# joshuaowalker/specimux

Hardware: AMD Instinct MI355X
Metric: reads/sec demultiplexed, 768-specimen ITS panel on 765k ONT-style reads (higher is better)
Workload: dtype u32

## Files before the change

### specimux_amd/csrc/smx_demux_tile.h

```cpp
#ifndef SMX_DEMUX_TILE_H
#define SMX_DEMUX_TILE_H
#include <hip/hip_runtime.h>
#include <stdint.h>
#include "smx_internal.h"
#include "smx_barcode_core.h"
#include "smx_align_core.h"
#include "smx_scorer.h"

namespace smx {

__device__ inline void wave_exclusive_scan(unsigned short *a, int n) {
    int lane = threadIdx.x & 63;
    int chunk = (n + 63) / 64;
    int lo = lane * chunk, hi = lo + chunk < n ? lo + chunk : n;
    int sum = 0;
    for (int i = lo; i < hi; i++) sum += a[i];
    int incl = sum;
    for (int d = 1; d < 64; d <<= 1) {
        int v = __shfl_up(incl, d, 64);
        if (lane >= d) incl += v;
    }
    int run = incl - sum;
    for (int i = lo; i < hi; i++) { int v = a[i]; a[i] = (unsigned short)run; run += v; }
    if (lane == 63) a[n] = (unsigned short)incl;
}

__device__ __forceinline__ int nth_location(const unsigned *mrow, int MW, int jstar, int loc_ord) {
    int seen = 0;
    for (int w = jstar >> 5; w < MW; w++) {
        unsigned word = mrow[w];
        if (w == (jstar >> 5)) word &= ~0u << (jstar & 31);
        int pc = __popc(word);
        if (seen + pc > loc_ord) {
            for (int t = loc_ord - seen; t > 0; t--) word &= word - 1;
            return w * 32 + __ffs(word) - 1;
        }
        seen += pc;
    }
    return -1;
}


template <typename PW, int NT, int BSV, int CM, int SP>
struct DemuxTile {
    static constexpr bool sp = SP != 0;
    static constexpr bool cmode = CM == 1;
    static constexpr bool redo = CM == 2;
    static constexpr int PWBITS = (int)sizeof(PW) * 8;
    unsigned char *lds;
    const DevPanel *P;
    const uint8_t *windows;
    const int32_t *lens;
    uint32_t n_reads;
    smx_op *ops, *extra;
    uint32_t extra_cap;
    uint32_t *n_extra;
    unsigned long long *counts;
    smx_hit *dbg_hits;
    int8_t *dbg_bdist;
    unsigned *tile_counter;
    const unsigned *pre;
    DemuxAux aux;
    int R, NP, NB, S, H, MW, maxB, need_starts, n_pbc, NPAIR, npmeta, use_slots, use_bs, ncand;
    TileLayout T;
    int CS, NPs, NBs, lNPs, lNBs, G, logG, MBW;
    int stride, kidx, pfmin, preorient, minlen, maxlen, lH, SW;
    unsigned Hmagic, hcmagic;
    uint32_t redo_ratio, n_tiles;
    bool cfilt, timing;
    unsigned long long *tacc, *dbg_phase;
    PW *ppeq, *prpeq;
    unsigned *bpeq, *bsre;
    unsigned char *lut, *codes;
    unsigned *namask;
    int *lensL, *ocnt;
    HitL *hits;
    unsigned *masks, *tieb, *bres, *dmask;
    int tstr;
    EntL *ents;
    int *etail;
    unsigned short *offsA, *offsB;
    unsigned short *queue;
    int *cumL;
    smx_op *opsL;
    int *aggr;
    unsigned short *hmap, *clist;
    unsigned long long *pmask, *hcand;
    LPanel LP;
    int tid, wave;
    uint32_t cur, r0, nxt;
    int par, nr, nh, nI;
    bool live;
    unsigned popped;
    bool pop_issued;
    int *lensC, *ocntC;
    bool prelisted;
    int nq, nE_pre;

    __device__ __forceinline__ void workgroup_done() {
        __builtin_amdgcn_fence(__ATOMIC_RELEASE, "workgroup");
        const unsigned prev = atomicAdd(tile_counter + 2, 1u);
        if (prev == gridDim.x - 1) {
            __threadfence();
            tile_counter[0] = 0; tile_counter[2] = 0;
            if (!cmode) {
                *n_extra = atomicAdd(tile_counter + 3, 0u);
                tile_counter[1] = 0; tile_counter[3] = 0;
            }
        }
    }
    __device__ __forceinline__ int divH(int x) const { return lH >= 0 ? (x >> lH) : (int)__umulhi((unsigned)x, Hmagic); }
    __device__ __forceinline__ void tile_span(uint32_t t, uint32_t &first, int &count) const {
        if (!redo) {
            first = t * (uint32_t)R;
            count = (int)((n_reads - first) < (uint32_t)R ? (n_reads - first) : (uint32_t)R);
        } else {
            const uint32_t seg = t / redo_ratio, sub = t - seg * redo_ratio;
            const uint32_t base = aux.ovf_list[seg] * (uint32_t)aux.Rc;
            const uint32_t end = base + (uint32_t)aux.Rc < n_reads ? base + (uint32_t)aux.Rc : n_reads;
            first = base + sub * (uint32_t)R;
            count = first < end ? (int)((end - first) < (uint32_t)R ? (end - first) : (uint32_t)R) : 0;
            if (count == 0) first = base;
        }
    }
    __device__ __forceinline__ void stamp(int i) {
        asm volatile("" : "+v"(tid));
        if (timing) { unsigned long long _t = clock64(); tacc[i] += _t - tacc[10]; tacc[10] = _t; }
    }

    __device__ __forceinline__ void pop_tile() {
        if (tid == 0) {
            unsigned off = 0;
            asm volatile("" : "+v"(off));
            popped = atomicAdd(tile_counter + off, 1u);
        }
        pop_issued = true;
    }

    __device__ __forceinline__ bool setup(unsigned char *lds_, const DevPanel *P_, const uint8_t *windows_, const int32_t *lens_,
                                          uint32_t n_reads_, int R_arg, smx_op *ops_, smx_op *extra_, uint32_t extra_cap_,
                                          uint32_t *n_extra_, unsigned long long *counts_, smx_hit *dbg_hits_, int8_t *dbg_bdist_arg,
                                          unsigned *tile_counter_, int use_slots_arg, const unsigned *pre_, const DemuxAux &aux_) {
        lds = lds_; P = P_; windows = windows_; lens = lens_; n_reads = n_reads_; ops = ops_; extra = extra_; extra_cap = extra_cap_;
        n_extra = n_extra_; counts = counts_; dbg_hits = dbg_hits_; tile_counter = tile_counter_; pre = pre_; aux = aux_;
        R = SP == 3 ? 32 : (SP == 2 ? SMX_SP2_R : (sp ? 64 : R_arg));
        NP = SP == 2 ? 2 : P->NP; NB = P->NB; S = SP == 3 ? 160 : (sp ? 80 : P->S); H = 2 * NP; MW = (S + 31) / 32; maxB = P->maxB;
        need_starts = sp ? 0 : P->need_starts;
        n_pbc = P->n_pbc; NPAIR = SP == 2 ? 1 : P->NPAIR;
        const LayoutArgs la = layout_args(NP, NB, n_pbc, NPAIR, P->trim);
        npmeta = la.npmeta;
        use_slots = SP != 0 ? 0 : use_slots_arg;
        dbg_bdist = SP != 0 ? nullptr : dbg_bdist_arg;
        use_bs = SP != 0 ? 1 : ((BSV != 0 && P->bs_ok && !use_slots) ? 1 : 0);
        ncand = la.ncand;
        const int tails = sp ? 0 : la.tails;
        T = make_layout<PW>(NP, NB, S, R, maxB, need_starts, npmeta, sp ? 3 : P->kidx, use_slots, P->bs_ok, ncand,
                            sp ? 0 : P->cap_hits, sp ? 0 : P->cap_ents, (sp && CM == 1) ? 256 : aux.nitems, tails, P->n_bstab);
        ppeq = (PW *)(lds + T.ppeq);
        prpeq = (PW *)(lds + T.prpeq);
        bpeq = (unsigned *)(lds + T.bpeq);
        bsre = (unsigned *)(lds + T.bsre);
        lut = lds + T.lut;
        codes = lds + T.codes;
        namask = (unsigned *)(lds + T.namask);
        lensL = (int *)(lds + T.lens);
        ocnt = (int *)(lds + T.ocnt);
        hits = (HitL *)(lds + T.hits);
        masks = (unsigned *)(lds + T.masks);
        if (layout_tie_in_rec(T.MBW, use_slots, tails)) { tieb = (unsigned *)(lds + T.hits); tstr = (int)(sizeof(HitL) / 4); }
        else { tieb = (unsigned *)(lds + T.tiem); tstr = sp ? 1 : T.MBW; }
        bres = (unsigned *)(lds + T.bres);
        dmask = (unsigned *)(lds + T.dmask);
        ents = (EntL *)(lds + T.ents);
        etail = (int *)(lds + T.etail);
        offsA = (unsigned short *)(lds + T.offsA);
        offsB = (unsigned short *)(lds + T.offsB);
        queue = (unsigned short *)(lds + T.queue);
        cumL = (int *)(lds + T.emit);
        opsL = (smx_op *)(lds + T.opsL);
        aggr = (int *)(lds + T.aggr);
        hmap = (unsigned short *)(lds + T.hmap);
        clist = (unsigned short *)(lds + T.clist);
        pmask = (unsigned long long *)(lds + T.pmask);
        hcand = (unsigned long long *)(lds + T.hcand);
        cfilt = layout_cfilt(H, NPAIR * 2);
        tid = threadIdx.x;
        wave = tid >> 6;
        if (redo && tile_counter[1] == 0) {
            if (tid == 0) workgroup_done();
            return false;
        }
        CS = T.CS; NPs = T.NPs; NBs = T.NBs; lNPs = T.lNPs; lNBs = T.lNBs; G = T.G; logG = T.logG; MBW = sp ? 1 : T.MBW;
        stride = SP == 3 ? 320 : (sp ? 160 : P->wstride);
        kidx = sp ? 3 : P->kidx; pfmin = P->pfmin;
        preorient = sp ? 1 : P->preorient; minlen = sp ? -1 : P->minlen; maxlen = sp ? -1 : P->maxlen;
        lH = (H & (H - 1)) == 0 ? 31 - __clz(H) : -1;
        Hmagic = (unsigned)((0x100000000ull + (unsigned)H - 1) / (unsigned)H);
        hcmagic = (unsigned)((0x100000000ull + (unsigned)(S >> 4) - 1) / (unsigned)((S >> 4) > 0 ? (S >> 4) : 1));
        redo_ratio = redo ? (uint32_t)((aux.Rc + R - 1) / R) : 1u;
        n_tiles = redo ? tile_counter[1] * redo_ratio : (n_reads + R - 1) / R;
        tacc = (unsigned long long *)(lds + T.tacc);
        dbg_phase = sp ? nullptr : P->dbg_phase;
        timing = dbg_phase != nullptr && tid == 0;
        SW = (R + 63) >> 6;
        return true;
    }

    __device__ __forceinline__ void stage_panel() {
        for (int i = tid; i < NP * 16; i += NT) {
            int p = i >> 4, c = i & 15;
            ppeq[c * NPs + p] = (PW)P->ppeq[i] << (PWBITS - P->pm[p]);
            if (need_starts) prpeq[c * NPs + p] = (PW)P->prpeq[i];
        }
        if (!use_bs)
            for (int i = tid; i < NB * 16; i += NT) bpeq[(i & 15) * NBs + (i >> 4)] = P->bpeq[i];
        if (use_bs)
            for (int i = tid; i < P->n_bstab * T.MBW * 256; i += NT) {
                int blk = i >> 8;
                bsre[blk * T.BSP + (i & 255)] = P->bs_re[i];
            }
        for (int i = tid; i < 512; i += NT) lut[i] = P->lut[i];
        int *pmeta = (int *)(lds + T.pmeta);
        {
            int *q = pmeta;
            LP.pm = q; q += NP; LP.pk = q; q += NP; LP.pdir = q; q += NP; LP.pfidx = q; q += NP;
            LP.pbc_off = q; q += NP + 1; LP.pbc = q; q += n_pbc; LP.bm = q; q += NB;
            LP.pair_f = q; q += NPAIR; LP.pair_r = q; q += NPAIR; LP.pair_pool = q; q += NPAIR;
            LP.bstab = q;
            for (int i = tid; i < NP; i += NT) q[i] = P->bs_tab[i];
            for (int i = tid; i < NP; i += NT) {
                pmeta[i] = P->pm[i]; pmeta[NP + i] = P->pk[i]; pmeta[2 * NP + i] = P->pdir[i]; pmeta[3 * NP + i] = P->pfidx[i];
            }
            for (int i = tid; i <= NP; i += NT) pmeta[4 * NP + i] = P->pbc_off[i];
            for (int i = tid; i < n_pbc; i += NT) pmeta[5 * NP + 1 + i] = P->pbc[i];
            for (int i = tid; i < NB; i += NT) pmeta[5 * NP + 1 + n_pbc + i] = P->bm[i];
            for (int i = tid; i < NPAIR; i += NT) {
                int *b = pmeta + 5 * NP + 1 + n_pbc + NB;
                b[i] = P->pair_f[i]; b[NPAIR + i] = P->pair_r[i]; b[2 * NPAIR + i] = P->pair_pool[i];
            }
        }
        if (tid < 12) aggr[tid] = 0;
        if (cfilt) for (int i = tid; i < R; i += NT) pmask[i] = 0ull;
        if (cfilt) for (int i = tid; i < H; i += NT) hcand[i] = 0ull;
        if (cmode && tid == 0) {
            HitL hn;
            hn.tail_end = -1; hn.nloc = 0; hn.ntied = 0; hn.first_tied = -1; hn.pdist = -1; hn.bbest = -2; hn.jstar = 0; hn.fs_j = 0;
            hn.flags = 0; hn.pad = 0;
            hits[T.NI] = hn;
            for (int w = 0; w < T.MBW; w++) tieb[T.NI * tstr + w] = 0;
        }
        __syncthreads();
        if (cfilt)
            for (int ci = tid; ci < NPAIR * 2; ci += NT) {
                const int pair = ci >> 1, o = ci & 1;
                const int h1 = LP.pair_f[pair] * 2 + (o == 0 ? 0 : 1), h2 = LP.pair_r[pair] * 2 + (o == 0 ? 1 : 0);
                atomicOr(&hcand[h1], 1ull << ci);
                atomicOr(&hcand[h2], 1ull << ci);
            }
        __syncthreads();

        if (timing) for (int i = 0; i < 11; i++) tacc[i] = 0;
    }

    __device__ __forceinline__ void primer_item(int item, const bool use_pre) {
        const int dn = cmode ? (int)clist[item] : item;
        int r = divH(dn), h = dn - __mul24(r, H), p = h >> 1, X = h & 1;
        int L = lensC[r];
        EndGeom g = end_geom(L, S);
        const unsigned char *cw = codes + __mul24(r * 2 + X, CS);
        const PW *peq = ppeq + p;
        const int m = LP.pm[p], k = LP.pk[p], top = PWBITS - 1;
        PW Pvv = ~(PW)0, Mv = 0;
        int score = m, best = m + 1, jstar = 0, cnt = 0;
        unsigned *mrow = masks + __mul24(item, MW);
        bool pre_done = false, pre_omatch = false;
        if (use_pre) {
            const uint32_t gr = r0 + (uint32_t)r;
            const unsigned *pw = pre + ((size_t)(gr >> 10) * H + h) * (S >> 4) * PRE_TILE + (gr & (PRE_TILE - 1));
            const int bfull = S == 160 ? prescan_decode<10>(pw, PRE_TILE, 10, MW, m, k, g.Sp, mrow, &jstar, &cnt)
                            : S == 80 ? prescan_decode<5>(pw, PRE_TILE, 5, MW, m, k, g.Sp, mrow, &jstar, &cnt)
                                      : prescan_decode<0>(pw, PRE_TILE, S >> 4, MW, m, k, g.Sp, mrow, &jstar, &cnt);
            pre_omatch = bfull <= k;
            if (g.j_lo == 0) { pre_done = true; best = pre_omatch ? bfull : m + 1; }
            else { jstar = 0; cnt = 0; }
        }
        if (pre_done) {
        } else if (sizeof(PW) == 4 && g.j_lo == 0 && g.Sp == S && (S & 3) == 0) {
            const unsigned *pq = (const unsigned *)ppeq + p;
            unsigned Pu = ~0u, Mu = 0;
            int sc = m, bst = m + 1;
            const int esh = lNPs + 2;
#define SMX_PCOL(J) do { const unsigned e_ = *(const unsigned *)((const char *)pq + ((unsigned)cw[J] << esh)); \
                     myers_step_hw_top(e_, Pu, Mu, sc);                                              \
                     ltw = __builtin_amdgcn_alignbit(ltw, (unsigned)(sc - bst), 31);                  \
                     gtw = __builtin_amdgcn_alignbit(gtw, (unsigned)(bst - sc), 31);                  \
                     bst = sc < bst ? sc : bst; } while (0)
            for (int w = 0; w < MW; w++) {
                const int ncols = S - w * 32 < 32 ? S - w * 32 : 32;
                unsigned gtw = 0, ltw = 0;
                int j = w * 32;
                const int jend = j + ncols;
                for (; j + 8 <= jend; j += 8) {
                    SMX_PCOL(j); SMX_PCOL(j + 1); SMX_PCOL(j + 2); SMX_PCOL(j + 3);
                    SMX_PCOL(j + 4); SMX_PCOL(j + 5); SMX_PCOL(j + 6); SMX_PCOL(j + 7);
                }
                if (j < jend) { SMX_PCOL(j); SMX_PCOL(j + 1); SMX_PCOL(j + 2); SMX_PCOL(j + 3); }
                if (ncols > 0) {
                    mrow[w] = __brev(~gtw) >> (32 - ncols);
                    if (ltw) jstar = w * 32 + ncols - __ffs(ltw);
                } else mrow[w] = 0;
            }
#undef SMX_PCOL
            best = bst; score = sc;
            Pvv = (PW)Pu; Mv = (PW)Mu;
            for (int w = jstar >> 5; w < MW; w++) {
                unsigned word = mrow[w];
                if (w == (jstar >> 5)) word &= ~0u << (jstar & 31);
                cnt += __popc(word);
            }
        } else if (g.j_lo == 0) {
            const int Sp = g.Sp;
            for (int w = 0; w < MW; w++) {
                unsigned word = 0;
                int jend = (w + 1) * 32 < Sp ? (w + 1) * 32 : Sp;
#pragma unroll 4
                for (int j = w * 32; j < jend; j++) {
                    myers_step<PW, false>(peq[(int)cw[j] << lNPs], Pvv, Mv, score, top);
                    bool lt = score < best;
                    best = lt ? score : best;
                    jstar = lt ? j : jstar;
                    word |= (score == best ? 1u : 0u) << (j & 31);
                }
                mrow[w] = word;
            }
            for (int w = jstar >> 5; w < MW; w++) {
                unsigned word = mrow[w];
                if (w == (jstar >> 5)) word &= ~0u << (jstar & 31);
                cnt += __popc(word);
            }
        } else {
            for (int w = 0; w < MW; w++) mrow[w] = 0;
            for (int j = g.j_lo; j < g.Sp; j++) {
                myers_step<PW, false>(peq[(int)cw[j] << lNPs], Pvv, Mv, score, top);
                if (score < best) { best = score; jstar = j; cnt = 0; }
                if (score == best) { cnt++; mrow[j >> 5] |= 1u << (j & 31); }
            }
        }
        bool matched = best <= k;
        bool omatch = matched;
        if (g.j_lo > 0 && use_pre) omatch = pre_omatch;
        else if (g.j_lo > 0) {
            PW P2 = ~(PW)0, M2 = 0;
            int sc = m, b2 = m + 1;
            for (int j = 0; j < g.Sp; j++) {
                myers_step<PW, false>(peq[(int)cw[j] << lNPs], P2, M2, sc, top);
                b2 = sc < b2 ? sc : b2;
            }
            omatch = b2 <= k;
        }
        int fs_j = jstar;
        if (matched && need_starts) {
            const PW *rpeq = prpeq + p;
            PW P2 = ~(PW)0, M2 = 0;
            int sc = m, lastc = 1;
            int maxc = m + best;
            for (int c = 1; c <= maxc; c++) {
                int j = jstar - (c - 1);
                if (j < g.j_lo) break;
                myers_step<PW, true>(rpeq[(int)cw[j] << lNPs], P2, M2, sc, m - 1);
                if (sc == best) lastc = c;
            }
            fs_j = jstar - (lastc - 1);
        }
        HitL hl;
        hl.tail_end = -1;
        hl.pdist = (signed char)(matched ? best : -1);
        hl.nloc = (short)(matched ? cnt : 0);
        hl.bbest = -2; hl.ntied = 0; hl.first_tied = -1;
        hl.jstar = (unsigned char)jstar; hl.fs_j = (unsigned char)fs_j;
        hl.flags = (unsigned char)(omatch ? 1 : 0); hl.pad = 0;
        hits[item] = hl;
        if (cfilt && matched) atomicOr(&pmask[r], 1ull << h);
        if (omatch) {
            int dir = LP.pdir[p];
            int vote_fwd = (dir == 0) ? (X == 0) : (X == 1);
            atomicAdd(&ocntC[r], vote_fwd ? 1 : 0x10000);
        }
    }

    __device__ __forceinline__ void phase2_primers() {
        unsigned short *fbq = queue;
        if (cmode) {
            for (int i0 = tid; i0 < nh; i0 += 4 * NT) {
                unsigned mw[4];
#pragma unroll
                for (int u = 0; u < 4; u++) {
                    const int i = i0 + u * NT < nh ? i0 + u * NT : nh - 1;
                    const int r = divH(i), h = i - __mul24(r, H);
                    const uint32_t gr = r0 + (uint32_t)r;
                    mw[u] = aux.match[((size_t)(gr >> 10) * H + h) * PRE_G + ((gr & (PRE_TILE - 1)) >> 5)] >> (gr & 31);
                }
#pragma unroll
                for (int u = 0; u < 4; u++) {
                    const int i = i0 + u * NT;
                    if (i < nh) {
                        const bool flagged = (mw[u] & 1u) || (ocntC[divH(i)] & OCNT_NA) != 0;
                        int rec = T.NI;
                        if (flagged) {
                            const int sl = atomicAdd(&aggr[11], 1);
                            if (sl < T.NI) { clist[sl] = (unsigned short)i; rec = sl; }
                        }
                        hmap[i] = (unsigned short)rec;
                    }
                }
            }
            __syncthreads();
            nI = aggr[11];
            if (nI > T.NI) {
                live = false;
                if (tid == 0) aux.ovf_list[atomicAdd(tile_counter + 1, 1u)] = cur;
            }
        }
        if (!live) {
        } else if (pre != nullptr) {
            for (int item = tid; item < nI; item += NT) {
                if ((ocntC[divH(cmode ? (int)clist[item] : item)] & OCNT_NA) == 0) primer_item(item, true);
                else fbq[atomicAdd(&aggr[10], 1)] = (unsigned short)item;
            }
            __syncthreads();
            const int nfb = aggr[10];
            if (nfb > 0) {
                for (int i = tid; i < nfb; i += NT) primer_item((int)fbq[i], false);
                __syncthreads();
                if (tid == 0) aggr[10] = 0;
            }
        } else {
            for (int item = tid; item < nI; item += NT) primer_item(item, false);
            __syncthreads();
        }

    }

    __device__ __forceinline__ int locations_needed(int item) {
        const int dn = cmode ? (int)clist[item] : item;
        int r = divH(dn), h = dn - __mul24(r, H), p = h >> 1, X = h & 1;
        int L = lensC[r];
        int f = ocntC[r] & 0x7FFF, rv = ocntC[r] >> 16;
        int ori = 3;
        if (preorient) { if (f > 0 && rv == 0) ori = 1; else if (rv > 0 && f == 0) ori = 2; }
        bool filtered = (minlen != -1 && L < minlen) || (maxlen != -1 && L > maxlen);
        int dir = LP.pdir[p];
        bool in_fwd = (dir == 0) ? (X == 0) : (X == 1);
        bool needed = !filtered && ((in_fwd && (ori & 1)) || (!in_fwd && (ori & 2)));
        HitL &hl = hits[item];
        int n = 0;
        if (needed && hl.pdist >= 0) {
            hl.flags |= 2;
            hl.bbest = -1;
            n = hl.nloc;
        }
        for (int w = 0; w < MBW; w++) tieb[__mul24(item, tstr) + w] = 0;
        return n;
    }
    __device__ __forceinline__ void list_entries(int item, int rank_in_round, int e) {
        const int dn = cmode ? (int)clist[item] : item;
        int r = divH(dn), h = dn - __mul24(r, H), X = h & 1;
        const HitL &hl = hits[item];
        int L = lensC[r];
        EndGeom g = end_geom(L, S);
        const unsigned *mrow = masks + __mul24(item, MW);
        const unsigned *na = namask + __mul24(r * 2 + X, MW);
        int ord = 0;
        for (int w = hl.jstar >> 5; w < MW; w++) {
            unsigned word = mrow[w];
            if (w == (hl.jstar >> 5)) word &= ~0u << (hl.jstar & 31);
            while (word) {
                int je = w * 32 + __ffs(word) - 1;
                word &= word - 1;
                int bstart = (je - g.j_lo) + g.shift + 1;
                BcGeom bg = bc_geom(L, g.base, bstart);
                int ncol = g.Sp - bg.tj0;
                bool ok = ncol > 0;
                if (ok && pfmin > 0) {
                    if (!bg.pf_same || ncol < pfmin) ok = false;
                    else {
                        int wi = bg.tj0 >> 5, sh = bg.tj0 & 31;
                        unsigned long long two = ((unsigned long long)(wi + 1 < MW ? na[wi + 1] : 0u) << 32) | na[wi];
                        if ((two >> sh) & ((1ull << pfmin) - 1ull)) ok = false;
                    }
                }
                EntL en;
                en.hit = (unsigned short)item;
                en.slot = (unsigned short)(rank_in_round << logG);
                en.tj0 = (unsigned char)(ok ? bg.tj0 : 0);
                en.loc_ord = (unsigned char)ord;
                en.ncol = (unsigned char)(ncol > 255 ? 255 : (ncol < 0 ? 0 : ncol));
                en.ok = ok ? 1 : 0;
                en.delta = (short)bg.delta; en.pad = 0;
                ents[e++] = en;
                ord++;
            }
        }
    }

    __device__ __forceinline__ void phase3a_entries() {
        if (dbg_bdist)
            for (int i = tid; i < nh * maxB; i += NT) dbg_bdist[(size_t)r0 * H * maxB + i] = -1;
        prelisted = false;
        nq = 0; nE_pre = 0;
        if (nI <= NT) {
            const int item = tid;
            const int n = item < nI ? locations_needed(item) : 0;
            const unsigned pk = (unsigned)n | ((n > 0 ? 1u : 0u) << 16);
            unsigned incl = pk;
            for (int d = 1; d < 64; d <<= 1) {
                unsigned v = (unsigned)__shfl_up((int)incl, d, 64);
                if ((tid & 63) >= d) incl += v;
            }
            unsigned *wsum = (unsigned *)offsB;
            if ((tid & 63) == 63) wsum[wave] = incl;
            __syncthreads();
            unsigned base = 0, total = 0;
            for (int w = 0; w < NT / 64; w++) { unsigned v = wsum[w]; total += v; base += w < wave ? v : 0u; }
            const unsigned excl = base + incl - pk;
            nq = (int)(total >> 16);
            const int totE = (int)(total & 0xFFFFu);
            if (nq <= T.CAPH && totE <= T.CAPE) {
                prelisted = true;
                nE_pre = totE;
                if (n > 0) {
                    queue[excl >> 16] = (unsigned short)item;
                    if (BSV == 3) offsA[item] = (unsigned short)(excl & 0xFFFFu);
                    list_entries(item, (int)(excl >> 16), (int)(excl & 0xFFFFu));
                }
                if (use_slots) { for (int i = tid; i < (nq << logG); i += NT) bres[i] = 0xFFFFFFFFu; }
                else { for (int i = tid; i < nq * (kidx + 1) * MBW; i += NT) dmask[i] = 0; }
                __syncthreads();
            } else {
                __syncthreads();
                if (item < nI) {
                    offsA[item] = (unsigned short)(excl & 0xFFFFu);
                    offsB[item] = (unsigned short)(excl >> 16);
                    if (n > 0) queue[excl >> 16] = (unsigned short)item;
                }
                if (tid == 0) { offsA[nI] = (unsigned short)totE; offsB[nI] = (unsigned short)nq; }
                __syncthreads();
            }
        } else {
            for (int item = tid; item < nI; item += NT) {
                int n = locations_needed(item);
                offsA[item] = (unsigned short)n;
                offsB[item] = n > 0 ? 1 : 0;
            }
            __syncthreads();
            if (wave == 0) wave_exclusive_scan(offsA, nI);
            else if (wave == 1) wave_exclusive_scan(offsB, nI);
            __syncthreads();
            for (int item = tid; item < nI; item += NT)
                if (offsB[item + 1] != offsB[item]) queue[offsB[item]] = (unsigned short)item;
            nq = offsB[nI];
            __syncthreads();
        }

    }

    __device__ __forceinline__ void phase3b_barcodes(int nE) {
        if (BSV != 0 && use_bs) {
            const int bsm = P->bs_m;
            for (int item = tid; item < nE * MBW; item += NT) {
                int ei = item, w = 0;
                if (MBW != 1) { ei = item / MBW; w = item - ei * MBW; }
                const EntL en = ents[ei];
                if (BSV == 3) etail[ei] = -0x7FFFFFFF;
                if (!en.ok) continue;
                const int hh = cmode ? (int)clist[en.hit] : (int)en.hit, r = divH(hh), h = hh - __mul24(r, H), p = h >> 1, X = h & 1;
                const unsigned char *cwt = codes + __mul24(r * 2 + X, CS) + en.tj0;
                unsigned *dm = dmask + __mul24(__mul24(en.slot >> logG, kidx + 1), MBW) + w;
                if constexpr (BSV == 3) {
                    unsigned seen[4], ML[4];
                    const unsigned want[4] = {~0u, ~0u, ~0u, ~0u};
                    int tc = -1;
// ... 214 lines not shown
                else {
                    if (tid == 0) aggr[8] = q0 + 1;
                    __syncthreads();
                    for (int q = q0 + 2 + tid; q <= nq && q - q0 <= T.CAPH; q += NT) {
                        const int hq = queue[q - 1];
                        if (offsA[hq] + hits[hq].nloc - e_base <= T.CAPE) atomicMax(&aggr[8], q);
                    }
                    __syncthreads();
                    q1 = aggr[8];
                }
                const int e_end = (q1 < nq) ? offsA[queue[q1]] : offsA[nI];
                nE = e_end - e_base;
                for (int q = q0 + tid; q < q1; q += NT) {
                    int item = queue[q];
                    list_entries(item, q - q0, offsA[item] - e_base);
                }
                if (use_slots) { for (int i = tid; i < ((q1 - q0) << logG); i += NT) bres[i] = 0xFFFFFFFFu; }
                else { for (int i = tid; i < (q1 - q0) * (kidx + 1) * MBW; i += NT) dmask[i] = 0; }
                __syncthreads();
            }
            stamp(3);
            if (!pop_issued) pop_tile();
            phase3b_barcodes(nE);
            __syncthreads();
            stamp(4);
            phase3c_summary(q0, q1, e_base);
            __syncthreads();
            stamp(5);
            q0 = q1;
        }
    }

    __device__ __forceinline__ void zero_for_next() {
        for (int i = tid; i < R * 2 * MW; i += NT) namask[i] = 0;
        for (int i = tid; i < R; i += NT) ocnt[(par ^ 1) * R + i] = 0;
        if (live) for (int i = tid; i < nr * ncand; i += NT) cumL[i] = 0;
        if (tid == 0) { aggr[9] = (int)popped; aggr[11] = 0; }
        __syncthreads();
        nxt = (uint32_t)aggr[9];

    }

    __device__ __forceinline__ void phase4_score() {
        unsigned long long t_sc0 = 0;
        if (timing) t_sc0 = clock64();
        const int lG = R <= 16 ? 2 : (R <= 32 ? 1 : 0), G = 1 << lG;
        const int r = tid >> lG, sub = tid & (G - 1);
        if (r < nr) {
            int L = lensC[r];
            bool filtered = (minlen != -1 && L < minlen) || (maxlen != -1 && L > maxlen);
            const unsigned long long pm_r = cfilt ? pmask[r] : 0ull;
            if (cfilt && sub == 0) pmask[r] = 0ull;
            if (sub == 0) atomicAdd(&aggr[0], 1);
            if (filtered) {
                if (sub == 0) {
                    atomicAdd(&aggr[2], 1);
                    smx_op op;
                    op.sample = -1; op.trim_start = 0; op.trim_end = 0; op.pool = -1; op.p1 = op.p2 = -1; op.barcode = -1;
                    op.dist[0] = op.dist[1] = op.dist[2] = op.dist[3] = -1;
                    op.rtype = SMX_R_FILTERED; op.flags = 0; op.n_ops = 0; op.read = r0 + r;
                    opsL[r] = op;
                }
            } else {
                ReadCtx c;
                c.P = P; c.LP = LP; c.MBW = MBW; c.L = L; c.S = S;
                c.trim = sp ? (int)SMX_TRIM_BARCODES : P->trim; c.derep = sp ? (int)SMX_DEREP_BEST : P->derep;
                c.npair = NPAIR;
                c.tstr = tstr;
                if (cmode) { c.hits = hits; c.tiem = tieb; c.hmap = hmap + r * H; }
                else { c.hits = hits + r * H; c.tiem = tieb + r * H * tstr; c.hmap = nullptr; }
                c.hcand = cfilt ? hcand : nullptr;
                c.pm = pm_r;
                c.g = end_geom(L, S);
                int f = ocntC[r] & 0x7FFF, rv = ocntC[r] >> 16;
                int ori = 3;
                if (preorient) { if (f > 0 && rv == 0) ori = 1; else if (rv > 0 && f == 0) ori = 2; }
                c.set_live(ori);
                Emitter E;
                E.c = &c; E.primary = opsL + r; E.extra = extra; E.extra_cap = extra_cap;
                E.n_extra = tile_counter + 3;
                E.counts = counts; E.cum = cumL + r * ncand; E.aggr = aggr; E.read = r0 + r;
                E.n = 0; E.matched = false; E.overflow = false;
                const bool done = score_fast(E, ori, sub, G);
                if (sub == 0) {
                    if (!done) score_general(E, ori);
                    opsL[r].n_ops = (uint16_t)E.n;
                    if (E.matched) atomicAdd(&aggr[1], 1);
                    if (E.n > 1) atomicAdd(&aggr[6], 1);
                    if (E.overflow) atomicAdd(&aggr[7], 1);
                }
            }
        }
        if (timing) tacc[9] += clock64() - t_sc0;

    }

    __device__ __forceinline__ void phase1_encode() {
        const int wid = live ? tid - 64 * SW : tid, nw = live ? NT - 64 * SW : NT;
        const bool timing_enc = dbg_phase != nullptr && tid == 64 * SW;
        unsigned long long t_enc0 = 0;
        if (timing_enc) t_enc0 = clock64();
        uint32_t r0n;
        int nrn;
        tile_span(nxt, r0n, nrn);
        int *lensN = lensL + (par ^ 1) * R;
        int len_n = 0;
        bool have_len = false;
        auto load_len = [&](int r_item) {
            unsigned off = r0n + (uint32_t)(wid < nrn ? wid : r_item);
            asm volatile("" : "+v"(off));
            return lens[off];
        };
        auto encode_bytes = [&](int r, int L, int cpos, const uint4 &v) {
            int Sp = L < S ? L : S;
            unsigned w[4] = {v.x, v.y, v.z, v.w};
            unsigned char *rowA = codes + (r * 2 + 0) * CS, *rowB = codes + (r * 2 + 1) * CS;
            for (int b = 0; b < 16; b++) {
                int pos = cpos + b;
                unsigned ch = (w[b >> 2] >> ((b & 3) * 8)) & 0xFF;
                if (pos < S) {
                    if (pos < Sp) {
                        unsigned cd = lut[256 + ch];
                        int j = Sp - 1 - pos;
                        rowA[j] = (unsigned char)cd;
                        if (cd > 3) { atomicOr(&namask[(r * 2 + 0) * MW + (j >> 5)], 1u << (j & 31)); atomicOr(&ocnt[(par ^ 1) * R + r], OCNT_NA); }
                    }
                } else if (pos < 2 * S) {
                    int j = pos - S;
                    if (j < Sp) {
                        unsigned cd = lut[ch];
                        rowB[j] = (unsigned char)cd;
                        if (cd > 3) { atomicOr(&namask[(r * 2 + 1) * MW + (j >> 5)], 1u << (j & 31)); atomicOr(&ocnt[(par ^ 1) * R + r], OCNT_NA); }
                    }
                }
            }
        };
        if ((S & 15) == 0 && (sp || aux.codes2 != nullptr)) {
            const int hc = S >> 4, per = 2 * hc;
            const bool tiled = SP == 2 ? true : aux.tiled != 0;
            auto fast = [&](int r, int end, int c, unsigned z) {
                unsigned *dst = (unsigned *)(codes + __mul24(r * 2 + end, CS)) + 4 * c;
#pragma unroll
                for (int q = 0; q < 4; q++) {
                    const unsigned x = (z >> (2 * q)) & 0x03030303u;
                    dst[q] = x ^ ((x >> 1) & 0x01010101u);
                }
            };
            auto slow = [&](int r, int end, int c) {
                const uint4 v = *(const uint4 *)(windows + (size_t)(r0n + r) * stride + (end ? S : 0) + 16 * c);
                encode_bytes(r, lens[r0n + r], (end ? S : 0) + 16 * c, v);
            };
            if (tiled && ((r0n | (uint32_t)nrn) & 3u) == 0) {
                const int nq = nrn >> 2;
                for (int ci = wid; ci < per * 16; ci += nw) {
                    const int run = ci >> 4, r = (ci & 15) * 4;
                    len_n = load_len(0);
                    have_len = true;
                    if ((ci & 15) >= nq) continue;
                    const int end = run >= hc ? 1 : 0, c = run - (end ? hc : 0);
                    uint4 z4 = *(const uint4 *)(aux.codes2 + tilecodes_word((size_t)(r0n + r), hc, end, c));
                    unsigned f4 = *(const unsigned *)(aux.naflag + r0n + r);
                    asm volatile("" : "+v"(z4.x), "+v"(z4.y), "+v"(z4.z), "+v"(z4.w), "+v"(f4), "+v"(len_n));
                    if (!(f4 & 0xFFu)) fast(r, end, c, z4.x);
                    if (!(f4 & 0xFF00u)) fast(r + 1, end, c, z4.y);
                    if (!(f4 & 0xFF0000u)) fast(r + 2, end, c, z4.z);
                    if (!(f4 & 0xFF000000u)) fast(r + 3, end, c, z4.w);
                    if (f4) {
#pragma nounroll
                        for (int j = 0; j < 4; j++)
                            if ((f4 >> (8 * j)) & 0xFFu) slow(r + j, end, c);
                    }
                }
            } else {
                const unsigned permagic = (unsigned)((0x100000000ull + (unsigned)per - 1) / (unsigned)per);
                const int nci = tiled ? per * 64 : nrn * per;
                auto item_of = [&](int ci, int &r, int &end, int &c) {
                    int rem;
                    if (tiled) { r = ci & 63; rem = ci >> 6; }
                    else { r = (int)__umulhi((unsigned)ci, permagic); rem = ci - __mul24(r, per); }
                    end = rem >= hc ? 1 : 0; c = rem - (end ? hc : 0);
                    return ci < nci && r < nrn;
                };
                for (int ci0 = wid; ci0 < nci; ci0 += 4 * nw) {
                    unsigned z[4], fl[4];
#pragma unroll
                    for (int u = 0; u < 4; u++) {
                        const int ci = ci0 + u * nw;
                        int r, end, c;
                        if (!item_of(ci, r, end, c)) r = end = c = 0;
                        z[u] = aux.codes2[tiled ? tilecodes_word((size_t)(r0n + r), hc, end, c) : (size_t)r0n * per + (size_t)(__mul24(r, per) + end * hc + c)];
                        fl[u] = aux.naflag[r0n + r];
                        if (u == 0) len_n = load_len(r);
                    }
                    have_len = true;
                    asm volatile("" : "+v"(z[0]), "+v"(z[1]), "+v"(z[2]), "+v"(z[3]), "+v"(fl[0]), "+v"(fl[1]), "+v"(fl[2]), "+v"(fl[3]), "+v"(len_n));
                    unsigned slow_u = 0;
#pragma unroll
                    for (int u = 0; u < 4; u++) {
                        int r, end, c;
                        if (!item_of(ci0 + u * nw, r, end, c)) continue;
                        if (!fl[u]) fast(r, end, c, z[u]);
                        else slow_u |= 1u << u;
                    }
#pragma nounroll
                    for (; slow_u; slow_u &= slow_u - 1u) {
                        int r, end, c;
                        item_of(ci0 + (__ffs((int)slow_u) - 1) * nw, r, end, c);
                        slow(r, end, c);
                    }
                }
            }
        } else if (!sp && (S & 15) == 0) {
            const int hc = S >> 4, nhead = nrn * hc, S4 = S >> 2;
            for (int ci = wid; ci < 2 * nhead; ci += nw) {
                const bool tail = ci >= nhead;
                const int k = tail ? ci - nhead : ci;
                const int r = hc == 1 ? k : (int)__umulhi((unsigned)k, hcmagic), c = k - __mul24(r, hc);
                const uint4 v = *(const uint4 *)(windows + (size_t)(r0n + r) * stride + (tail ? S : 0) + 16 * c);
                const int L = lens[r0n + r];
                const unsigned w[4] = {v.x, v.y, v.z, v.w};
                unsigned pk[4];
                bool acgt = L >= S;
#pragma unroll
                for (int q = 0; q < 4; q++) {
                    const unsigned x = (w[q] >> 1) & 0x03030303u;
                    const unsigned y = x ^ ((x >> 1) & 0x01010101u);
                    acgt = acgt && (__builtin_amdgcn_perm(0u, 0x54474341u, y) == w[q]);
                    pk[q] = tail ? y : __builtin_amdgcn_perm(0u, y ^ 0x03030303u, 0x00010203u);
                }
                if (acgt) {
                    unsigned *dst = (unsigned *)(codes + __mul24(r * 2 + (tail ? 1 : 0), CS));
#pragma unroll
                    for (int q = 0; q < 4; q++) dst[tail ? 4 * c + q : S4 - 1 - (4 * c + q)] = pk[q];
                } else {
                    encode_bytes(r, L, (tail ? S : 0) + 16 * c, v);
                }
            }
        } else if (!sp) {
            const int chunks = stride / 16;
            const uint4 *src = (const uint4 *)(windows + (size_t)r0n * stride);
            for (int ci = wid; ci < nrn * chunks; ci += nw) {
                int r = ci / chunks;
                encode_bytes(r, lens[r0n + r], (ci - r * chunks) * 16, src[ci]);
            }
        }
        if (wid < nrn) {
            if (!have_len) len_n = lens[r0n + wid];
            lensN[wid] = len_n;
        }
        if (timing_enc) tacc[8] += clock64() - t_enc0;
    }

    __device__ __forceinline__ void phase5_store() {
        if (live) {
            const uint4 *srcv = (const uint4 *)opsL;
            uint4 *dstv = (uint4 *)(ops + r0);
            for (int i = tid; i < nr * 2; i += NT) dstv[i] = srcv[i];
        }
        if (live && dbg_hits) {
            for (int item = tid; item < nh; item += NT) {
                int r = divH(item);
                const HitL &hl = hits[cmode ? (int)hmap[item] : item];
                EndGeom g = end_geom(lensC[r], S);
                smx_hit o;
                o.pdist = hl.pdist; o.nloc = hl.nloc;
                o.first_start = hl.pdist >= 0 ? (int)hl.fs_j - g.j_lo + g.shift : -1;
                o.first_end = hl.pdist >= 0 ? (int)hl.jstar - g.j_lo + g.shift : -1;
                o.bbest = hl.bbest; o.ntied = hl.ntied;
                o.first_tied = (short)((hl.bbest >= 0) ? LP.pbc[LP.pbc_off[(item - r * H) >> 1] + hl.first_tied] : -1);
                o.tail_end = (hl.bbest >= 0 && tstr != (int)(sizeof(HitL) / 4)) ? hl.tail_end : -1;
                o.flags = (int16_t)(hl.flags & 1);
                dbg_hits[(size_t)(r0 + r) * H + (item - r * H)] = o;
            }
        }
        if (dbg_hits) __syncthreads();

    }

    __device__ __forceinline__ void run() {
        cur = 0xFFFFFFFFu;
        par = 1;
        for (;;) {
            asm volatile("" : "+v"(tid));
            const bool have = cur != 0xFFFFFFFFu;
            popped = 0;
            pop_issued = false;
            r0 = 0u;
            nr = 0;
            if (have) tile_span(cur, r0, nr);
            nh = nr * H;
            nI = nh;
            live = have;
            lensC = lensL + par * R; ocntC = ocnt + par * R;
            if (timing) tacc[10] = clock64();
            if (have) {
                phase2_primers();
                stamp(1);
                if (live) {
                    phase3a_entries();
                    stamp(2);
                    phase3_rounds();
                }
            }
            if (!pop_issued) pop_tile();
            zero_for_next();
            stamp(0);
            if (live && wave < SW) phase4_score();
            else if (nxt < n_tiles) phase1_encode();
            __syncthreads();
            stamp(6);
            phase5_store();
            stamp(7);
            if (nxt >= n_tiles) break;
            cur = nxt;
            par ^= 1;
        }
    }

    __device__ __forceinline__ void finish() {
        if (timing)
            for (int i = 0; i < 10; i++) dbg_phase[(size_t)blockIdx.x * 16 + i] += tacc[i];
        if (timing) dbg_phase[(size_t)blockIdx.x * 16 + 14] += tacc[0] != 0 || tacc[1] != 0 ? 1 : 0;
        if (dbg_phase != nullptr && (tid & 63) == 0)
            dbg_phase[(size_t)blockIdx.x * 16 + 10 + wave] = __builtin_amdgcn_s_getreg(4 | (0 << 6) | (31 << 11));
    #undef STAMP
        if (tid < 8 && aggr[tid]) atomicAdd(&counts[tid], (unsigned long long)aggr[tid]);
        __syncthreads();
        if (tid == 0) workgroup_done();

    }
};

template <typename PW, int NT, int BSV, int CM = 0, int SP = 0>
__global__ __launch_bounds__(NT, SP == 2 ? SMX_SP2_WG : 4) void demux_kernel(DevPanel Pv, const uint8_t *__restrict__ windows,
                                                    const int32_t *__restrict__ lens, uint32_t n_reads, int R_arg,
                                                    smx_op *__restrict__ ops, smx_op *__restrict__ extra,
                                                    uint32_t extra_cap, uint32_t *n_extra,
                                                    unsigned long long *counts, smx_hit *dbg_hits, int8_t *dbg_bdist_arg,
                                                    unsigned *tile_counter, int use_slots_arg,
                                                    const unsigned *__restrict__ pre, uint32_t npad, DemuxAux aux) {
    extern __shared__ __attribute__((aligned(16))) unsigned char lds[];
    (void)npad;
    DemuxTile<PW, NT, BSV, CM, SP> D;
    if (!D.setup(lds, &Pv, windows, lens, n_reads, R_arg, ops, extra, extra_cap, n_extra, counts, dbg_hits, dbg_bdist_arg,
                 tile_counter, use_slots_arg, pre, aux))
        return;
    D.stage_panel();
    D.run();
    D.finish();
}

}
#endif
```

### specimux_amd/csrc/smx_prescan_core.h

```cpp
#ifndef SMX_PRESCAN_CORE_H
#define SMX_PRESCAN_CORE_H
#include <stdint.h>

#include "smx_hd.h"
#include "smx_bitslice_core.h"

namespace smx {

constexpr int PRE_G = 32;
constexpr int PRE_TILE = PRE_G * 32;
constexpr int PRE_MAXROWS = 31;
constexpr int PRE_MAXSYM = 8;
constexpr int PRE_BLK = 33;
constexpr int PRE_SUBG = 8;
constexpr int PRE_CS = 291;
static_assert(PRE_CS >= PRE_SUBG * PRE_BLK && PRE_CS % 32 == 3, "staging stride");
constexpr int PRE_SCRATCH = 2 * (PRE_MAXSYM + 1) * 64;

struct PreDesc {
    int NP, S, nsym, pure4;
    uint8_t m[64], k[64];
    uint8_t symmask[64][PRE_MAXSYM];
    uint8_t sym[64][32];
};

SMX_HD unsigned perm_b32(unsigned a, unsigned b, unsigned sel) {
#if defined(__HIP_DEVICE_COMPILE__)
    return __builtin_amdgcn_perm(a, b, sel);
#else
    unsigned r = 0;
    for (int i = 0; i < 4; i++) {
        const unsigned q = (sel >> (8 * i)) & 7u;
        r |= (((q & 4u) ? a : b) >> (8 * (q & 3u)) & 0xFFu) << (8 * i);
    }
    return r;
#endif
}

SMX_HD unsigned bfi_b32(unsigned mask, unsigned a, unsigned b) {
#if defined(__HIP_DEVICE_COMPILE__)
    unsigned r;
    asm("v_bfi_b32 %0, %1, %2, %3" : "=v"(r) : "s"(mask), "v"(a), "v"(b));
    return r;
#else
    return (a & mask) | (b & ~mask);
#endif
}

template <int J>
SMX_HD void transpose32_pair(unsigned &lo, unsigned &hi) {
    const unsigned l = lo, h = hi;
    if (J == 16) {
        lo = perm_b32(h, l, 0x05040100u);
        hi = perm_b32(h, l, 0x07060302u);
    } else if (J == 8) {
        lo = perm_b32(h, l, 0x06020400u);
        hi = perm_b32(h, l, 0x07030501u);
    } else {
        constexpr unsigned M = J == 4 ? 0x0F0F0F0Fu : (J == 2 ? 0x33333333u : 0x55555555u);
        lo = bfi_b32(M, l, h << J);
        hi = bfi_b32(M, l >> J, h);
    }
}
SMX_HD void transpose32_fields(unsigned (&a)[32]) {
#define SMX_TSTAGE(J) _Pragma("unroll") for (int k_ = 0; k_ < 32; k_++) if ((k_ & J) == 0) transpose32_pair<J>(a[k_], a[k_ + J]);
    SMX_TSTAGE(16) SMX_TSTAGE(8) SMX_TSTAGE(4) SMX_TSTAGE(2) SMX_TSTAGE(1)
#undef SMX_TSTAGE
}
SMX_HD void transpose32(unsigned (&a)[32]) {
#if defined(__HIP_DEVICE_COMPILE__)
    transpose32_fields(a);
#else
#define SMX_TSTAGE(J, MASK)                                                                    \
    _Pragma("unroll") for (int k_ = 0; k_ < 32; k_++) if ((k_ & J) == 0) {                     \
        const unsigned t_ = ((a[k_] >> J) ^ a[k_ + J]) & MASK;                                 \
        a[k_ + J] ^= t_;                                                                       \
        a[k_] ^= t_ << J;                                                                      \
    }
    SMX_TSTAGE(16, 0x0000FFFFu)
    SMX_TSTAGE(8, 0x00FF00FFu)
    SMX_TSTAGE(4, 0x0F0F0F0Fu)
    SMX_TSTAGE(2, 0x33333333u)
    SMX_TSTAGE(1, 0x55555555u)
#undef SMX_TSTAGE
#endif
}

SMX_HD unsigned pack16(unsigned w0, unsigned w1, unsigned w2, unsigned w3) {
    unsigned z = (w0 >> 1) & 0x03030303u;
    z |= (w1 << 1) & 0x0C0C0C0Cu;
    z |= (w2 << 3) & 0x30303030u;
    z |= (w3 << 5) & 0xC0C0C0C0u;
    return z;
}
SMX_HD int pack_t(int q) { return 4 * ((q & 7) >> 1) + (q >> 3); }
SMX_HD int pack_pl(int q) { return q & 1; }

SMX_HD unsigned pack16_revcomp(unsigned z) {
#if defined(__HIP_DEVICE_COMPILE__)
    z = __builtin_amdgcn_perm(0u, z, 0x00010203u);
#else
    z = (z >> 24) | ((z >> 8) & 0xFF00u) | ((z << 8) & 0xFF0000u) | (z << 24);
#endif
    z = ((z & 0x0F0F0F0Fu) << 4) | ((z >> 4) & 0x0F0F0F0Fu);
    z = ((z & 0x33333333u) << 2) | ((z >> 2) & 0x33333333u);
    return z ^ 0xAAAAAAAAu;
}
SMX_HD unsigned acgt_mismatch(unsigned w) {
    const unsigned x = (w >> 1) & 0x03030303u;
#if defined(__HIP_DEVICE_COMPILE__)
    return __builtin_amdgcn_perm(0u, 0x47544341u, x) ^ w;
#else
    static const unsigned char L[4] = {'A', 'C', 'T', 'G'};
    unsigned r = 0;
    for (int i = 0; i < 4; i++) r |= (unsigned)L[(x >> (8 * i)) & 3] << (8 * i);
    return r ^ w;
#endif
}

SMX_HD size_t codes2_word(size_t read, int CH, int end, int chunk) { return (read * 2 + (size_t)end) * (size_t)CH + (size_t)chunk; }
SMX_HD unsigned codes2_from_piece(unsigned z, int c, int CH, int *end, int *chunk) {
    if (c < CH) { *end = 0; *chunk = CH - 1 - c; return pack16_revcomp(z); }
    *end = 1; *chunk = c - CH;
    return z;
}

SMX_HD size_t tilecodes_word(size_t read, int CH, int end, int chunk) {
    return (((read / PRE_TILE) * 2 + (size_t)end) * (size_t)CH + (size_t)chunk) * PRE_TILE + read % PRE_TILE;
}
SMX_HD constexpr int tile_bit(int t, int pl) { return 8 * (t & 3) + 2 * (t >> 2) + pl; }
constexpr int PRE_TS = PRE_SUBG * 32 + 4;
static_assert(PRE_TS % 4 == 0 && PRE_TS % 32 == 4, "staging stride of the tile-codes kernel");
SMX_HD void prescan_stage_code(unsigned *stage, int read_in_sub, int c, int CH, unsigned w0, unsigned w1, unsigned w2, unsigned w3) {
    int end, chunk;
    const unsigned zz = codes2_from_piece(pack16(w0, w1, w2, w3), c, CH, &end, &chunk);
    stage[(end * CH + chunk) * PRE_TS + read_in_sub] = zz;
}
SMX_HD void prescan_copy_codes(const unsigned *stage, unsigned *dst, int i) {
    constexpr int per = PRE_SUBG * 8;
    const int run = i / per, r4 = (i % per) * 4;
#if defined(__HIP_DEVICE_COMPILE__)
    *(uint4 *)(dst + (size_t)run * PRE_TILE + r4) = *(const uint4 *)(stage + run * PRE_TS + r4);
#else
    for (int j = 0; j < 4; j++) dst[(size_t)run * PRE_TILE + r4 + j] = stage[run * PRE_TS + r4 + j];
#endif
}

template <int CHT>
SMX_HD int prescan_decode(const unsigned *w, size_t cstride, int CH, int MW, int m, int k, int n_valid, unsigned *mrow,
                          int *jstar_out, int *nloc_out) {
    unsigned short *mrow16 = (unsigned short *)mrow;
    int nlt = 0, jstar = 0;
    auto chunk = [&](int c, unsigned xraw) {
        const int nv = n_valid - 16 * c;
        const unsigned keep = nv >= 16 ? 0xFFFFu : (nv > 0 ? (1u << nv) - 1u : 0u);
        const unsigned x = xraw & (keep | (keep << 16));
        const unsigned lt16 = x & 0xFFFFu;
#if defined(__HIP_DEVICE_COMPILE__)
        nlt += __popc(lt16);
        if (lt16) jstar = 16 * c + 31 - __clz((int)lt16);
#else
        nlt += __builtin_popcount(lt16);
        if (lt16) jstar = 16 * c + 31 - __builtin_clz(lt16);
#endif
        mrow16[c] = (unsigned short)(x >> 16);
    };
    if (CHT > 0) {
        unsigned xs[CHT > 0 ? CHT : 1];
#pragma unroll
        for (int c = 0; c < CHT; c++) xs[c] = w[(size_t)c * cstride];
#pragma unroll
        for (int c = 0; c < CHT; c++) chunk(c, xs[c]);
        CH = CHT;
    } else {
        for (int c0 = 0; c0 < CH; c0 += 4) {
            unsigned xs[4];
#pragma unroll
            for (int u = 0; u < 4; u++) xs[u] = c0 + u < CH ? w[(size_t)(c0 + u) * cstride] : 0u;
#pragma unroll
            for (int u = 0; u < 4; u++) if (c0 + u < CH) chunk(c0 + u, xs[u]);
        }
    }
    if (CH & 1) mrow16[CH] = 0;
    const int best = m - nlt;
    int nloc = 0;
    if (best <= k) {
        for (int i = 0; i < MW; i++) {
            unsigned v = mrow[i];
            if (i < (jstar >> 5)) v = 0;
            else if (i == (jstar >> 5)) v &= ~0u << (jstar & 31);
            mrow[i] = v;
#if defined(__HIP_DEVICE_COMPILE__)
            nloc += __popc(v);
#else
            nloc += __builtin_popcount(v);
#endif
        }
    }
    *jstar_out = jstar;
    *nloc_out = nloc;
    return best;
}

SMX_HD unsigned prescan_store_piece(unsigned *planes, int read_in_sub, int c, unsigned w0, unsigned w1, unsigned w2, unsigned w3) {
    const int g = read_in_sub >> 5, rr = read_in_sub & 31;
    const unsigned z = pack16(w0, w1, w2, w3);
    planes[c * PRE_CS + g * PRE_BLK + rr] = z;
    return z;
}

SMX_HD void prescan_short_head_piece(const uint8_t *row, int c, int S, int L, unsigned (&w)[4]) {
    const int sh = S - (L < 0 ? 0 : L);
    const int x0 = 16 * c - sh;
    const int base = x0 & ~3, sh8 = (x0 & 3) * 8;
    unsigned d[5];
#pragma unroll
    for (int k = 0; k < 5; k++) {
        const int idx = base + 4 * k;
        const int cl = idx < 0 ? 0 : (idx > S - 4 ? S - 4 : idx);
        const unsigned v = *(const unsigned *)(row + cl);
        d[k] = (idx >= 0 && idx <= S - 4) ? v : 0u;
    }
#pragma unroll
    for (int k = 0; k < 4; k++) w[k] = sh8 ? (d[k] >> sh8) | (d[k + 1] << (32 - sh8)) : d[k];
}

SMX_HD void prescan_transpose_block(const unsigned *planes, int g, int c, int CH, unsigned (&out)[32]) {
    unsigned a[32];
    const unsigned *pb = planes + c * PRE_CS + g * PRE_BLK;
#pragma unroll
    for (int r = 0; r < 32; r++) a[r] = pb[r];
    transpose32(a);
    const bool endA = c < CH;
#pragma unroll
    for (int d = 0; d < 32; d++) {
        const int tB = d >> 1, tA = 15 - (d >> 1), pl = d & 1;
        const unsigned wB = a[8 * (tB & 3) + 2 * (tB >> 2) + pl];
        const unsigned wA = pl ? ~a[8 * (tA & 3) + 2 * (tA >> 2) + pl] : a[8 * (tA & 3) + 2 * (tA >> 2) + pl];
        out[d] = endA ? wA : wB;
    }
}
SMX_HD int prescan_block_chunk(int c, int CH) { return c < CH ? CH - 1 - c : c - CH; }
SMX_HD int prescan_block_lane(int g, int c, int CH) { return g * 2 + (c < CH ? 0 : 1); }
SMX_HD size_t prescan_plane_word(int chunk, int lane, int d) { return ((size_t)chunk * 64 + lane) * 32 + d; }

template <int NX>
SMX_HD void prescan_write_occ(unsigned *sc, unsigned b0, unsigned b1, const unsigned (&xm)[NX > 0 ? NX : 1][4]) {
    const unsigned E0 = ~b0 & ~b1, E1 = b0 & ~b1, E2 = ~b0 & b1, E3 = b0 & b1;
    sc[0] = E0; sc[64] = E1; sc[128] = E2; sc[192] = E3;
#pragma unroll
    for (int x = 0; x < NX; x++)
        sc[(4 + x) * 64] = (E0 & xm[x][0]) | (E1 & xm[x][1]) | (E2 & xm[x][2]) | (E3 & xm[x][3]);
}

template <int MR, int NX, int MT = 1, int TS = 0>
SMX_HD void prescan_dp(const unsigned *gpl, unsigned *scratch, int lane, int CH, const PreDesc &D, int p, unsigned *wout,
                       size_t cstride, unsigned *mout) {
    const int m = D.m[p], skip = MR - m;
    unsigned Pv[MR], Mv[MR];
    int aoff[MR];
#pragma unroll
    for (int i = 0; i < MR; i++) {
        Pv[i] = i >= skip ? ~0u : 0u; Mv[i] = 0u;
        aoff[i] = (i >= skip ? (int)D.sym[p][i - skip] : PRE_MAXSYM) * 64 + lane;
    }
    unsigned xm[NX > 0 ? NX : 1][4];
#pragma unroll
    for (int x = 0; x < (NX > 0 ? NX : 1); x++)
#pragma unroll
        for (int b = 0; b < 4; b++) xm[x][b] = ((D.symmask[p][4 + x] >> b) & 1) ? ~0u : 0u;
    unsigned g0 = 0, g1 = 0, g2 = 0, g3 = 0, g4 = 0, zero = ~0u;
    unsigned n0 = 0, n1 = 0, n2 = 0, n3 = 0, n4 = 0;
    constexpr int bufw = PRE_SCRATCH / 2;
    unsigned *sc0 = scratch + lane, *sc1 = scratch + bufw + lane;
    sc0[PRE_MAXSYM * 64] = ~0u; sc1[PRE_MAXSYM * 64] = ~0u;
    unsigned pw[2][8];
    unsigned tc[32], tn[32];
    auto tfetch = [&](int chunk, int q, unsigned (&dst)[32]) {
        const size_t at = ((size_t)((lane & 1) * CH + chunk)) * PRE_TILE + (size_t)(lane >> 1) * 32 + 4 * q;
#if defined(__HIP_DEVICE_COMPILE__)
        const uint4 u = *(const uint4 *)(gpl + at);
        dst[4 * q] = u.x; dst[4 * q + 1] = u.y; dst[4 * q + 2] = u.z; dst[4 * q + 3] = u.w;
#else
        for (int j = 0; j < 4; j++) dst[4 * q + j] = gpl[at + j];
#endif
    };
    auto fetch = [&](int grp, unsigned (&dst)[8]) {
        const int chunk = grp >> 2, q = (grp & 3) * 2;
#if defined(__HIP_DEVICE_COMPILE__)
        const uint4 *g4 = (const uint4 *)gpl;
        const uint4 u0 = g4[((size_t)chunk * 64 + lane) * 8 + q], u1 = g4[((size_t)chunk * 64 + lane) * 8 + q + 1];
        dst[0] = u0.x; dst[1] = u0.y; dst[2] = u0.z; dst[3] = u0.w; dst[4] = u1.x; dst[5] = u1.y; dst[6] = u1.z; dst[7] = u1.w;
#else
        for (int j = 0; j < 8; j++) dst[j] = gpl[prescan_plane_word(chunk, lane, 4 * q + j)];
#endif
    };
    if (TS) {
#pragma unroll
        for (int q = 0; q < 8; q++) tfetch(0, q, tc);
#pragma unroll
        for (int i = 0; i < 32; i++) tn[i] = 0u;
        transpose32(tc);
        prescan_write_occ<NX>(sc0, tc[tile_bit(0, 0)], tc[tile_bit(0, 1)], xm);
    } else {
        fetch(0, pw[0]);
        prescan_write_occ<NX>(sc0, pw[0][0], pw[0][1], xm);
    }
    unsigned eqb[2][8];
#pragma unroll
    for (int u = 0; u < 8; u++) eqb[0][u] = scratch[aoff[u]];
    for (int ch = 0; ch < CH; ch++) {
        unsigned fl[32];
#pragma unroll
        for (int t = 0; t < 16; t++) {
            const int gq = t >> 2, tq = t & 3, cur = gq & 1;
            unsigned *scw = (t & 1) ? sc0 : sc1;
            if (TS) {
                if (t < 8 && ch + 1 < CH) tfetch(ch + 1, t, tn);
                if (t == 15 && ch + 1 < CH) transpose32(tn);
                if (t < 15) prescan_write_occ<NX>(scw, tc[tile_bit((t + 1) & 15, 0)], tc[tile_bit((t + 1) & 15, 1)], xm);
                else if (ch + 1 < CH) prescan_write_occ<NX>(scw, tn[tile_bit(0, 0)], tn[tile_bit(0, 1)], xm);
            } else {
                if (tq == 0 && (ch * 4 + gq + 1 < CH * 4)) fetch(ch * 4 + gq + 1, pw[cur ^ 1]);
                if (tq < 3) prescan_write_occ<NX>(scw, pw[cur][2 * tq + 2], pw[cur][2 * tq + 3], xm);
                else if (ch * 4 + gq + 1 < CH * 4) prescan_write_occ<NX>(scw, pw[cur ^ 1][0], pw[cur ^ 1][1], xm);
            }
            const unsigned *sc = ((t & 1) ? scratch + bufw : scratch);
            unsigned Ph = 0u, Mh = 0u;
            constexpr int NG = (MR + 7) / 8;
#pragma unroll
            for (int gi = 0; gi < NG; gi++) {
                const int cur = (t * NG + gi) & 1;
                const int gn = gi + 1 < NG ? gi + 1 : 0;
                const unsigned *scn = gi + 1 < NG ? sc : ((t & 1) ? scratch : scratch + bufw);
#pragma unroll
                for (int u = 0; u < 8; u++) if (gn * 8 + u < MR) eqb[cur ^ 1][u] = scn[aoff[gn * 8 + u]];
#if defined(__HIP_DEVICE_COMPILE__)
                __builtin_amdgcn_sched_barrier(0);
#endif
#pragma unroll
                for (int u = 0; u < 8; u++) if (gi * 8 + u < MR) {
                    const int i = gi * 8 + u;
#if defined(__HIP_DEVICE_COMPILE__)
                    unsigned Z, nPh, nMh;
                    asm volatile("v_bitop3_b32 %[z], %[eq], %[mh], %[mv] bitop3:0xfe\n\t"
                                 "v_bitop3_b32 %[pho], %[mv], %[z], %[pv] bitop3:0xf1\n\t"
                                 "v_and_b32 %[mho], %[pv], %[z]\n\t"
                                 "v_bitop3_b32 %[pv], %[mh], %[z], %[ph] bitop3:0xf1\n\t"
                                 "v_and_b32 %[mv], %[ph], %[z]"
                                 : [z] "=&v"(Z), [pho] "=&v"(nPh), [mho] "=&v"(nMh), [pv] "+v"(Pv[i]), [mv] "+v"(Mv[i])
                                 : [eq] "v"(eqb[cur][u]), [mh] "v"(Mh), [ph] "v"(Ph));
                    Ph = nPh; Mh = nMh;
#else
                    const unsigned Z = eqb[cur][u] | Mh | Mv[i];
// ... 88 lines not shown
```

Before: 3.067 billion.

## Prefetch prescan flag words into registers during encode loop for SP2 tiles

During the tiled code-encode loop, each lane now also loads the five prescan flag words for its primer item into registers. It stages one 16-byte slice per lane into the shared dmask buffer. The primer phase then decodes from these registers or from shared memory instead of issuing strided global loads per item. The goal is to hide global-load latency in the primer scan behind the encode phase, at the cost of extra VGPRs and a one-item-per-lane assumption enforced by static_asserts.

```diff
diff --git a/specimux_amd/csrc/smx_demux_tile.h b/specimux_amd/csrc/smx_demux_tile.h
--- a/specimux_amd/csrc/smx_demux_tile.h
+++ b/specimux_amd/csrc/smx_demux_tile.h
@@ -96,6 +96,18 @@
     int *lensC, *ocntC;
     bool prelisted;
     int nq, nE_pre;
+    static constexpr bool pfx = SP == 2 && CM == 0;
+    static constexpr int PFX_LANES = 80;
+    static_assert(!pfx || (NT == 256 && SMX_SP2_R == 64 && PRE_TILE % SMX_SP2_R == 0), "flag-word prefetch: one item per lane, a tile inside one DP tile");
+    static_assert(!pfx || 2 * (80 >> 4) * 16 <= NT - 64, "flag-word prefetch: the 16-byte encode loop is one pass for every lane");
+    unsigned fw[5];
+    static_assert(sizeof(HitL) % 16 == 0, "flag-word prefetch: dmask takes 16-byte stores");
+    __device__ __forceinline__ bool flags_prefetched(uint32_t first, int count) const {
+        return pfx && ((first | (uint32_t)count) & 3u) == 0;
+    }
+    __device__ __forceinline__ void pin_flag_words(uint4 &s4) {
+        asm volatile("" : "+v"(fw[0]), "+v"(fw[1]), "+v"(fw[2]), "+v"(fw[3]), "+v"(fw[4]), "+v"(s4.x), "+v"(s4.y), "+v"(s4.z), "+v"(s4.w));
+    }
 
     __device__ __forceinline__ void workgroup_done() {
         __builtin_amdgcn_fence(__ATOMIC_RELEASE, "workgroup");
@@ -277,7 +289,22 @@
         if (use_pre) {
             const uint32_t gr = r0 + (uint32_t)r;
             const unsigned *pw = pre + ((size_t)(gr >> 10) * H + h) * (S >> 4) * PRE_TILE + (gr & (PRE_TILE - 1));
-            const int bfull = S == 160 ? prescan_decode<10>(pw, PRE_TILE, 10, MW, m, k, g.Sp, mrow, &jstar, &cnt)
+            int bfull;
+            if constexpr (pfx) {
+                unsigned xs[5];
+                if (!flags_prefetched(r0, nr)) {
+#pragma unroll
+                    for (int c = 0; c < 5; c++) xs[c] = pw[(size_t)c * PRE_TILE];
+                } else if (wave == 0) {
+#pragma unroll
+                    for (int c = 0; c < 5; c++) xs[c] = dmask[c * 64 + h * 16 + r];
+                } else {
+#pragma unroll
+                    for (int c = 0; c < 5; c++) xs[c] = fw[c];
+                }
+                bfull = prescan_decode_words<5>(xs, MW, m, k, g.Sp, mrow, &jstar, &cnt);
+            } else
+            bfull = S == 160 ? prescan_decode<10>(pw, PRE_TILE, 10, MW, m, k, g.Sp, mrow, &jstar, &cnt)
                             : S == 80 ? prescan_decode<5>(pw, PRE_TILE, 5, MW, m, k, g.Sp, mrow, &jstar, &cnt)
                                       : prescan_decode<0>(pw, PRE_TILE, S >> 4, MW, m, k, g.Sp, mrow, &jstar, &cnt);
             pre_omatch = bfull <= k;
@@ -423,10 +450,12 @@
         }
         if (!live) {
         } else if (pre != nullptr) {
-            for (int item = tid; item < nI; item += NT) {
+            auto scan_or_queue = [&](int item) {
                 if ((ocntC[divH(cmode ? (int)clist[item] : item)] & OCNT_NA) == 0) primer_item(item, true);
                 else fbq[atomicAdd(&aggr[10], 1)] = (unsigned short)item;
-            }
+            };
+            if constexpr (pfx) { if (tid < nI) scan_or_queue(tid); }
+            else for (int item = tid; item < nI; item += NT) scan_or_queue(item);
             __syncthreads();
             const int nfb = aggr[10];
             if (nfb > 0) {
@@ -947,15 +976,36 @@
             };
             if (tiled && ((r0n | (uint32_t)nrn) & 3u) == 0) {
                 const int nq = nrn >> 2;
-                for (int ci = wid; ci < per * 16; ci += nw) {
+                auto stage_flag_words = [&](uint4 &s4) {
+                    pin_flag_words(s4);
+                    if (wid < PFX_LANES && (wid & 3) < nq) {
+                        const unsigned srun = (unsigned)wid >> 2, h = srun / 5u, c = srun - 5u * h;
+                        *(uint4 *)(dmask + c * 64 + h * 16 + (wid & 3) * 4) = s4;
+                    }
+                };
+                for (int ci = wid; ci < (pfx ? nw : per * 16); ci += nw) {
                     const int run = ci >> 4, r = (ci & 15) * 4;
                     len_n = load_len(0);
                     have_len = true;
-                    if ((ci & 15) >= nq) continue;
+                    uint4 s4 = make_uint4(0u, 0u, 0u, 0u);
+                    if constexpr (pfx) {
+                        const unsigned *tw = pre + (size_t)(r0n >> 10) * (4 * 5 * PRE_TILE) + (r0n & (PRE_TILE - 1));
+                        unsigned off = tid < nrn * 4 ? (unsigned)((tid & 3) * (5 * PRE_TILE) + (tid >> 2)) : 0u;
+                        unsigned offs = wid < PFX_LANES && (wid & 3) < nq ? (unsigned)((wid >> 2) * PRE_TILE + (wid & 3) * 4) : 0u;
+                        asm volatile("" : "+v"(off), "+v"(offs));
+#pragma unroll
+                        for (int c = 0; c < 5; c++) fw[c] = tw[off + c * PRE_TILE];
+                        s4 = *(const uint4 *)(tw + offs);
+                    }
+                    if (ci >= per * 16 || (ci & 15) >= nq) {
+                        if constexpr (pfx) stage_flag_words(s4);
+                        continue;
+                    }
                     const int end = run >= hc ? 1 : 0, c = run - (end ? hc : 0);
                     uint4 z4 = *(const uint4 *)(aux.codes2 + tilecodes_word((size_t)(r0n + r), hc, end, c));
                     unsigned f4 = *(const unsigned *)(aux.naflag + r0n + r);
                     asm volatile("" : "+v"(z4.x), "+v"(z4.y), "+v"(z4.z), "+v"(z4.w), "+v"(f4), "+v"(len_n));
+                    if constexpr (pfx) stage_flag_words(s4);
                     if (!(f4 & 0xFFu)) fast(r, end, c, z4.x);
                     if (!(f4 & 0xFF00u)) fast(r + 1, end, c, z4.y);
                     if (!(f4 & 0xFF0000u)) fast(r + 2, end, c, z4.z);
@@ -1075,6 +1125,7 @@
     __device__ __forceinline__ void run() {
         cur = 0xFFFFFFFFu;
         par = 1;
+        for (int c = 0; c < 5; c++) fw[c] = 0u;
         for (;;) {
             asm volatile("" : "+v"(tid));
             const bool have = cur != 0xFFFFFFFFu;
@@ -1090,6 +1141,7 @@
             if (timing) tacc[10] = clock64();
             if (have) {
                 phase2_primers();
+                if (pfx) for (int c = 0; c < 5; c++) fw[c] = 0u;
                 stamp(1);
                 if (live) {
                     phase3a_entries();
diff --git a/specimux_amd/csrc/smx_prescan_core.h b/specimux_amd/csrc/smx_prescan_core.h
--- a/specimux_amd/csrc/smx_prescan_core.h
+++ b/specimux_amd/csrc/smx_prescan_core.h
@@ -146,10 +146,15 @@
 #endif
 }
 
+#if defined(__HIP_DEVICE_COMPILE__)
+typedef unsigned short prescan_u16;
+#else
+typedef unsigned short __attribute__((may_alias)) prescan_u16;
+#endif
 template <int CHT>
 SMX_HD int prescan_decode(const unsigned *w, size_t cstride, int CH, int MW, int m, int k, int n_valid, unsigned *mrow,
                           int *jstar_out, int *nloc_out) {
-    unsigned short *mrow16 = (unsigned short *)mrow;
+    prescan_u16 *mrow16 = (prescan_u16 *)mrow;
     int nlt = 0, jstar = 0;
     auto chunk = [&](int c, unsigned xraw) {
         const int nv = n_valid - 16 * c;
@@ -200,6 +205,12 @@
     *jstar_out = jstar;
     *nloc_out = nloc;
     return best;
+}
+template <int CHT>
+SMX_HD int prescan_decode_words(const unsigned (&xs)[CHT], int MW, int m, int k, int n_valid, unsigned *mrow, int *jstar_out,
+                                int *nloc_out) {
+    static_assert(CHT > 0, "the words-in form has a compile-time chunk count");
+    return prescan_decode<CHT>(xs, 1, CHT, MW, m, k, n_valid, mrow, jstar_out, nloc_out);
 }
 
 SMX_HD unsigned prescan_store_piece(unsigned *planes, int read_in_sub, int c, unsigned w0, unsigned w1, unsigned w2, unsigned w3) {
```

After: 3.126 billion, median of 6. +1.9%, better.
